# zkp-gravity/0g-halo2

Measured on AMD Instinct MI355X. Metric: create_proof proofs/hour, model_28input_256entry_1hash_1bpi, higher is better.
Workload: dtype u32x8 (254-bit Montgomery integers)

## Files before the change

### 0g-halo2_amd/csrc/field9.h

```cpp
#pragma once

#include "curve.h"
#include "field.h"

namespace zg {

struct F9 {
    int32_t l[9];
};

constexpr int32_t MASK29 = (1 << 29) - 1;

struct Fq9Params {
    static __device__ __forceinline__ int32_t p(int i) {
        constexpr int32_t P[9] = {0x187cfd47, 0x010460b6, 0x1c72a34f, 0x02d522d0, 0x1585d978,
                                  0x02db40c0, 0x00a6e141, 0x0e5c2634, 0x0030644e};
        return P[i];
    }
    static constexpr uint32_t INV29 = 0x04866389u;
    static __device__ __forceinline__ F9 one() {
        return F9{{0x157ccc21, 0x141c2758, 0x185230d3, 0x014c0419, 0x0aa36fb9, 0x1d4240ce, 0x11d54c07, 0x052ac7a8, 0x000dc836}};
    }
    static __device__ __forceinline__ F9 k256() {
        return F9{{0x058f0d9d, 0x1aea1c6e, 0x11c2cf74, 0x11d651eb, 0x1462c0a7, 0x11b7bc3c, 0x1cbd99ba, 0x183340fb, 0x000e0a77}};
// ... 284 lines not shown
        c = w >> 29;
    }
    a.l[8] = (int32_t)((int64_t)v.l[8] - (int64_t)q * (int64_t)P::p(8) + c);
    int32_t b = 0;
#pragma unroll
    for (int i = 0; i < 8; i++) {
        const int32_t w = a.l[i] - P::p(i) + b;
        t.l[i] = w & MASK29;
        b = w >> 29;
    }
    t.l[8] = a.l[8] - P::p(8) + b;
    const bool ge = t.l[8] >= 0;
#pragma unroll
    for (int i = 0; i < 9; i++) a.l[i] = ge ? t.l[i] : a.l[i];
    return f9_pack(a);
}

struct alignas(16) XYZZ9 {
    F9 x, y, zz, zzz;
};
static_assert(sizeof(XYZZ9) == 144, "XYZZ9 layout");

__device__ __forceinline__ XYZZ9 xyzz9_identity() {
    XYZZ9 r;
#pragma unroll
    for (int i = 0; i < 9; i++) r.x.l[i] = r.y.l[i] = r.zz.l[i] = r.zzz.l[i] = 0;
    return r;
}
__device__ __forceinline__ bool xyzz9_is_identity(const XYZZ9& a) { return f9_limbs_zero(a.zz); }

// ... 332 lines not shown
```

### 0g-halo2_amd/csrc/poly.h

```cpp
#pragma once

#include "common.h"
#include "msm.h"

namespace zg {

struct alignas(16) DMono {
    Fe coeff;
    uint32_t n_factors;
    uint32_t coeff_is_one;
    uint32_t factors[ZG_MAX_FACTORS];
    uint32_t pad[2];
};
static_assert(sizeof(DMono) == 80, "DMono layout");

struct DLookup {
    uint32_t width;
    zg_poly inputs[ZG_MAX_LOOKUP_WIDTH];
    zg_poly tables[ZG_MAX_LOOKUP_WIDTH];
};

struct DevCircuit {
    const zg_query* queries;
    const DMono* monos;
    const zg_poly* gates;
    const DLookup* lookups;
    const zg_query* perm_cols;
    uint32_t n_gates, n_lookups, n_perm, chunk, n_sets;
};

struct Cols {
    const Fe* fixed;
    const Fe* advice;
    const Fe* instance;
    uint32_t log_size;
    int32_t rot_scale;
    size_t adv_bs, inst_bs;
};

constexpr uint32_t PC_MAX_POINTS = 16;
constexpr uint32_t EH_MAX_YPOW = 48;
struct alignas(16) ProofConst {
    uint32_t key[8];
    Fe theta, beta, gamma;
    Fe eh_y, eh_beta, eh_gamma, eh_theta;
    Fe eh_delta_start[2];
    Fe eh_ypow[EH_MAX_YPOW];
    Fe xn;
    Fe v;
    Fe points[PC_MAX_POINTS];
    Fe subs[PC_MAX_POINTS];
};

struct EvalHArgs {
    DevCircuit c;
    Cols cols;
    const Fe* sigma_cos;
    const Fe* pz_cos;
    const Fe* lz_cos;
    const Fe* pin_cos;
    const Fe* ptab_cos;
    size_t perm_stride;
    const Fe* l0;
    const Fe* llast;
    const Fe* lactive;
    const Fe* ext_tw;
    const Fe* t_eval;
    uint32_t t_mask;
    int32_t last_rot;
    const ProofConst* pc;
    uint32_t zpow;
    size_t cos_bs, h_bs;
// ... 110 lines not shown
```

### 0g-halo2_amd/csrc/poly.hip

```cpp
#include "poly.h"
#include "poly_eval.h"
#include "field9.h"

namespace zg {

__host__ __device__ __forceinline__ uint32_t rotl32(uint32_t x, int sft) { return (x << sft) | (x >> (32 - sft)); }
#define ZG_QR(a, b, c, d)                       \
    do {                                        \
        a += b; d ^= a; d = rotl32(d, 16);      \
        c += d; b ^= c; b = rotl32(b, 12);      \
        a += b; d ^= a; d = rotl32(d, 8);       \
        c += d; b ^= c; b = rotl32(b, 7);       \
    } while (0)

__host__ __device__ inline Fe rand_fr(const uint32_t* key, uint32_t tag, uint64_t index) {
    Fe v;
    for (uint32_t attempt = 0;; attempt++) {
        uint32_t x0 = 0x61707865u, x1 = 0x3320646eu, x2 = 0x79622d32u, x3 = 0x6b206574u;
        uint32_t x4 = key[0], x5 = key[1], x6 = key[2], x7 = key[3], x8 = key[4], x9 = key[5], x10 = key[6], x11 = key[7];
        uint32_t x12 = attempt, x13 = tag, x14 = (uint32_t)index, x15 = (uint32_t)(index >> 32);
        for (int r = 0; r < 10; r++) {
            ZG_QR(x0, x4, x8, x12);
            ZG_QR(x1, x5, x9, x13);
            ZG_QR(x2, x6, x10, x14);
// ... 668 lines not shown
#pragma unroll
    for (int i = 0; i < 9; i++) acc.l[i] = 0;
    uint32_t pending = 0;
    auto add = [&](const F9& t, bool neg) {
        acc = neg ? f9_sub(acc, t) : f9_add(acc, t);
        if (++pending == 2) {
            acc = f9_norm(acc);
            pending = 0;
        }
    };
    F9 hl, hr;
    bool held = false, hneg = false;
    for (uint32_t m = p.first; m < p.first + p.count; m++) {
        const DMono* mo = monos + m;
        const uint32_t nf = mo->n_factors;
        const bool unit = mo->coeff_is_one != 0 && nf > 0;
        const bool neg = unit && mo->coeff_is_one == 2;
        const uint32_t terms = nf + (unit ? 0u : 1u);
        if (terms == 1) {
            add(unit ? cell(mo->factors[0]) : f9_unpack(mo->coeff), neg);
            continue;
        }
        uint32_t f = 0;
        F9 l = unit ? cell(mo->factors[f++]) : f9_unpack(mo->coeff);
        for (; f + 1 < nf; f++) l = Fr9::mul(l, cell(mo->factors[f]));
        const F9 r = cell(mo->factors[nf - 1]);
        if (held) {
            if (hneg == neg) add(Fr9::mul2<false>(hl, hr, l, r), neg);
            else add(Fr9::mul2<true>(hl, hr, l, r), hneg);
            held = false;
        } else {
            hl = l;
            hr = r;
            hneg = neg;
            held = true;
        }
    }
    if (held) add(Fr9::mul(hl, hr), hneg);
    return f9_norm(acc);
// ... 9 lines not shown
                                                           const Fe* __restrict__ coef, uint32_t count, Fe* __restrict__ out) {
    const uint32_t idx = blockIdx.x * blockDim.x + threadIdx.x;
    if (idx >= en) return;
    stg(out + idx, f9_reduce_pack<Fr9Params>(horner9(ld9(col + ((idx + rot_off) & (en - 1))), coef, count)));
}

int poly_gate_factor(zg_ctx* ctx, const Fe* col, uint32_t rot_off, uint32_t en, const Fe* coef, uint32_t count, Fe* out) {
    ZG_REQUIRE(count >= 1 && (en & (en - 1)) == 0, ZG_ERR_INVALID_ARG, "poly_gate_factor: %u coefficients, %u points", count, en);
    ZG_LAUNCH(ctx, "gate_factor", 2.0 * en * 32.0, gate_factor9_kernel, dim3((en + 255) / 256), dim3(256), 0, col, rot_off, en, coef,
              count, out);
    ZG_HIP(hipGetLastError());
    return ZG_OK;
}

template <bool GROUPED>
__global__ __launch_bounds__(256) void evaluate_h9_kernel(EvalHArgs a, uint32_t en) {
    const uint32_t idx = blockIdx.x * blockDim.x + threadIdx.x;
    if (idx >= en) return;
    const EvalHProof pr = evalh_proof(a, blockIdx.y);
    const ProofConst* pc = pr.pc;
    const DevCircuit& c = a.c;
    const uint32_t mask = en - 1;
    const uint32_t rs = (uint32_t)a.cols.rot_scale;
    const uint32_t r_next = (idx + rs) & mask;
    const uint32_t r_prev = (idx - rs) & mask;
    const uint32_t r_last = (idx + (uint32_t)(a.last_rot * (int32_t)rs)) & mask;
    auto fold = [&](const F9& value, const F9& term) { return f9_add(Fr9::mul(value, f9_unpack(pc->eh_y)), term); };
    auto fold2 = [&](const F9& value, const F9& u, const F9& v) { return Fr9::mul2<false>(value, f9_unpack(pc->eh_y), u, v); };
    F9 value;
#pragma unroll
    for (int i = 0; i < 9; i++) value.l[i] = 0;
    auto cell = [&](uint32_t qi) {
        const zg_query q = c.queries[qi];
        const Fe* base = q.kind == ZG_FIXED ? pr.cols.fixed : q.kind == ZG_ADVICE ? pr.cols.advice : pr.cols.instance;
// ... 40 lines not shown
        for (int i = 0; i < 9; i++) s0.l[i] = sl.l[i] = sa.l[i] = 0;
        auto acc1 = [&](F9& s, uint32_t e, const F9& t) { s = f9_norm(f9_add(s, Fr9::mul(yw(e), t))); };
        auto acc2 = [&](F9& s, uint32_t e, const F9& t, uint32_t e2, const F9& t2) {
            s = f9_norm(f9_add(s, Fr9::mul2<false>(yw(e), t, yw(e2), t2)));
        };
        if (c.n_sets > 0) {
            const F9 zf = ld9(pr.pz_cos + idx);
            const F9 zl = ld9(pr.pz_cos + (size_t)(c.n_sets - 1) * en + idx);
            acc1(s0, w - 1, f9_sub(one(), zf));
            acc1(sl, w - 2, f9_sub(Fr9::sqr(zl), zl));
            w -= 2;
            for (uint32_t s = 1; s < c.n_sets; s++) {
                const F9 t = f9_sub(ld9(pr.pz_cos + (size_t)s * en + idx), ld9(pr.pz_cos + (size_t)(s - 1) * en + r_last));
                acc1(s0, --w, t);
            }
            F9 current_delta = Fr9::mul(f9_unpack(pc->eh_delta_start[a.zpow - 1]), ld9(a.ext_tw + idx));
            const F9 delta = f9_unpack(a.delta);
            for (uint32_t s = 0; s < c.n_sets; s++) {
                uint32_t c0 = s * c.chunk, c1 = c0 + c.chunk;
                if (c1 > c.n_perm) c1 = c.n_perm;
                F9 left = ld9(pr.pz_cos + (size_t)s * en + r_next);
                F9 right = ld9(pr.pz_cos + (size_t)s * en + idx);
                for (uint32_t col = c0; col < c1; col++) {
                    const zg_query q = c.perm_cols[col];
                    const Fe* base = q.kind == ZG_FIXED ? pr.cols.fixed : q.kind == ZG_ADVICE ? pr.cols.advice : pr.cols.instance;
                    const F9 v = ld9(base + ((size_t)q.column << a.cols.log_size) + idx);
                    const F9 sg = ld9(a.sigma_cos + (size_t)col * en + idx);
                    const F9 fl = f9_norm(f9_add(f9_add(Fr9::mul(f9_unpack(pc->eh_beta), sg), v), f9_unpack(pc->eh_gamma)));
                    const F9 fr = f9_norm(f9_add(f9_add(v, current_delta), f9_unpack(pc->eh_gamma)));
                    current_delta = Fr9::mul(current_delta, delta);
                    if (col + 1 < c1) {
                        left = Fr9::mul(left, fl);
                        right = Fr9::mul(right, fr);
                    } else {
                        left = Fr9::mul2<true>(left, fl, right, fr);
                    }
                }
                acc1(sa, --w, left);
            }
        }
        for (uint32_t l = 0; l < c.n_lookups; l++) {
            const DLookup* lk = c.lookups + l;
            F9 ai, ti;
            compress(lk, ai, ti);
            const Fe* zc = pr.lz_cos + (size_t)l * en;
            const Fe* ap = pr.pin_cos + (size_t)l * a.perm_stride;
            const Fe* sp = pr.ptab_cos + (size_t)l * a.perm_stride;
            const F9 z = ld9(zc + idx), apv = ld9(ap + idx), spv = ld9(sp + idx);
            const F9 lft = Fr9::mul(f9_add(apv, f9_unpack(pc->eh_beta)), f9_norm(f9_add(spv, f9_unpack(pc->eh_gamma))));
            const F9 rgt = Fr9::mul(f9_norm(f9_add(ai, f9_unpack(pc->eh_beta))), f9_norm(f9_add(ti, f9_unpack(pc->eh_gamma))));
            const F9 ams = f9_sub(apv, spv);
            acc2(s0, w - 1, f9_sub(one(), z), w - 4, ams);
            acc1(sl, w - 2, f9_sub(Fr9::sqr(z), z));
// ... 57 lines not shown
    value = Fr9::mul(value, ld9(a.t_eval + (idx & a.t_mask)));
    stg(pr.h + idx, f9_reduce_pack<Fr9Params>(value));
}

int poly_evaluate_h(zg_ctx* ctx, const EvalHArgs& a, uint32_t en, uint32_t nb, uint32_t n_columns, double unit_share) {
    if (!nb) return ZG_OK;
    ZG_REQUIRE(a.pc != nullptr && (a.zpow == 1 || a.zpow == 2), ZG_ERR_INVALID_ARG, "evaluate_h: per-proof scalars missing");
    const DevCircuit& c = a.c;
    const double arrays = (double)n_columns + 3.0 + c.n_perm + c.n_sets + 3.0 * c.n_lookups + 1.0;
    const double unit = nb * arrays * unit_share * 32.0;
    ZG_REQUIRE(!a.hat || a.monos_hat != nullptr || (c.n_gates == 0 && c.n_lookups == 0), ZG_ERR_INVALID_ARG,
               "evaluate_h: the 2^261-form monomial table is missing");
    ZG_REQUIRE(!a.hat || c.n_gates == 0 || (a.gates_hat != nullptr && a.gate_common != nullptr && a.gate_uni != nullptr && a.uni_coef != nullptr && a.gate_slab != nullptr && a.gate_slabs != nullptr), ZG_ERR_INVALID_ARG,
               "evaluate_h: the factored gate table is missing");
    if (a.hat && a.n_terms)
        ZG_LAUNCH_U(ctx, "evaluate_h", nb * arrays * en * 32.0, unit, evaluate_h9_kernel<true>, dim3((en + 255) / 256, nb), dim3(256), 0, a, en);
    else if (a.hat)
        ZG_LAUNCH_U(ctx, "evaluate_h", nb * arrays * en * 32.0, unit, evaluate_h9_kernel<false>, dim3((en + 255) / 256, nb), dim3(256), 0, a, en);
    else
        ZG_LAUNCH_U(ctx, "evaluate_h", nb * arrays * en * 32.0, unit, evaluate_h_kernel, dim3((en + 255) / 256, nb), dim3(256), 0, a, en);
    ZG_HIP(hipGetLastError());
    return ZG_OK;
}

__device__ __forceinline__ const Fe* poly_of(const PolySet& ps, uint32_t ix, uint32_t b) {
    return ix < ps.nsh ? ps.sh + (size_t)ix * ps.n : ps.pp + (size_t)b * ps.pp_bs + (size_t)(ix - ps.nsh) * ps.n;
}

template <uint32_t CH>
__global__ __launch_bounds__(256) void powers_kernel(const ProofConst* __restrict__ pc, uint32_t n, Fe* __restrict__ pw,
                                                     size_t pw_bs) {
    uint32_t i0 = (blockIdx.x * blockDim.x + threadIdx.x) * CH;
    if (i0 >= n) return;
// ... 524 lines not shown
```

### 0g-halo2_amd/csrc/prove_batch.hip

```cpp
#include <algorithm>
#include <chrono>

#include "prover.h"
#include "field9.h"
#include "transcript.h"

using namespace zg;

namespace {

Fe rotate_omega(const PkDev& k, const Fe& x, int32_t rot) {
    Fe w = rot >= 0 ? Fr::pow_u64(k.omega, (uint64_t)rot) : Fr::pow_u64(k.omega_inv, (uint64_t)(-(int64_t)rot));
    return Fr::mul(x, w);
}

constexpr int LAT_GATE_DEFAULT = 0;
constexpr int LAT_PULL_DEFAULT = 1;
void* stage(zg_prover* p, const void* src, size_t bytes) {
    void* dst = p->pin.stage_take(bytes);
    if (dst) memcpy(dst, src, bytes);
    return dst;
}
int h2d_list(zg_prover* p, uint32_t* d_dst, const std::vector<uint32_t>& list) {
    std::vector<uint32_t>& held = p->uploaded_lists[d_dst];
// ... 509 lines not shown
        const uint32_t mb = S + NL;
        if (mb) {
            ZG_TRY(wait_points(p, (size_t)nb * prod_per, pts, W_PRODUCTS));
            ZG_TICK("products: points on the host");
            for (uint32_t b = 0; b < nb; b++) {
                const Jac* q = &pts[(size_t)b * prod_per];
                for (uint32_t i = 0; i < mb; i++) tr[b].write_point(q[i]);
                if (!have_random) random_commit[b] = q[mb];
            }
        } else if (!have_random) {
            ZG_TRY(wait_points(p, nb, pts, W_PRODUCTS));
            for (uint32_t b = 0; b < nb; b++) random_commit[b] = pts[b];
        }
        have_random = true;
        for (uint32_t b = 0; b < nb; b++) tr[b].write_point(random_commit[b]);
        for (uint32_t b = 0; b < nb; b++) evalh_consts(p->hpc[b], tr[b].squeeze(), hat, evalh_terms(pk));
        ZG_TICK("y");
        ZG_TRY(publish());
        ZG_TICK("y uploaded");
        lap(2);
        return ZG_OK;
    }

    int quotient_queue() {
        ZG_TRY(join());
        if (!phase_cosets) ZG_TRY(to_cosets(ctx, p->ix_adv, p->ncos));
        for (uint32_t di = dlo; di < dhi; di++) {
            const EvalHArgs a = evalh_args(p, di);
            ZG_TRY(poly_evaluate_h(ctx, a, pk.dom[di].en, nb, A + I + pk.F, (double)((size_t)1 << ek) * ((double)pk.dom[di].en / parts_en)));
        }
        p->have_last = true;
// ... 306 lines not shown
```

### 0g-halo2_amd/csrc/prover.h

```cpp
#pragma once

#include <memory>

#include "poly.h"
#include "check.h"

namespace zg {

struct PkDev {
    int device = 0;
    uint32_t k = 0, ext_k = 0, cs_degree = 0, bf = 0, qpd = 0;
    uint32_t n = 0, en = 0, usable = 0;
    uint32_t F = 0, A = 0, I = 0, P = 0, NL = 0, sets = 0, chunk = 0;
    std::vector<zg_query> advice_queries, fixed_queries;
    DevCircuit dc{};
    std::vector<void*> owned;
    bool hat = true;
    bool grouped = true;
    DMono* monos_hat = nullptr;
    zg_poly* gates_hat = nullptr;
    uint32_t* gate_common = nullptr;
    zg_poly* gate_uni = nullptr;
    Fe* uni_coef = nullptr;
    uint32_t* gate_slab = nullptr;
    struct SlabJob { uint32_t gate, query, first, count; };
    std::vector<SlabJob> slab_jobs;
    Fe vk_repr{};
    Fe omega{}, omega_inv{}, ifft_div{};
    Fe *fixed_val = nullptr, *sigma_val = nullptr, *omega_tw = nullptr;
    Fe* sh_polys = nullptr;
    struct Dom {
        uint32_t ek = 0, en = 0;
        int zpow = 1;
        Fe *fixed_cos = nullptr, *sigma_cos = nullptr, *l0 = nullptr, *llast = nullptr, *lactive = nullptr,
           *gate_slabs = nullptr, *t_eval = nullptr, *ext_tw = nullptr;
    };
    Dom dom[3];
    uint32_t nparts = 1;
    uint32_t NG = 0;
    CheckInfo ck;
    ~PkDev() {
        (void)hipSetDevice(device);
        for (void* q : owned) (void)hipFree(q);
    }
};

struct PinnedArena {
    static constexpr size_t MARGIN = 4096;
    char* host = nullptr;
// ... 75 lines not shown
    zg::PinnedArena pin;
    bool have_last = false;
    bool in_flight = false;
    bool last_split = false;
    uint32_t last_nb = 0;
    double phase_ms[8] = {0, 0, 0, 0, 0, 0, 0, 0};
};

namespace zg {

int prover_drain(zg_prover* p);
int batch_args_ok(const char* who, const char* what, const zg_prover* p, size_t count, const zg_fr* const* instance, size_t instance_len);
int advice_into_slots(zg_prover* p, uint32_t nb, const zg_fr* const* advice_host, void* const* advice_dev);
int upload_consts(zg_prover* p, uint32_t nb);
uint32_t evalh_terms(const PkDev& pk);
void evalh_consts(ProofConst& c, const Fe& y, bool hat, uint32_t n_terms);
EvalHArgs evalh_args(const zg_prover* p, uint32_t di);
int shard_gather_sum(zg_prover* p, size_t count, XYZZ* out);

}
```

### 0g-halo2_amd/csrc/prover.hip

```cpp
#include <algorithm>
#include <cstdlib>
#include <memory>

#include "prover.h"
#include "field9.h"

using namespace zg;

namespace {

constexpr int LAT_SPLIT_K_DEFAULT = 15;

template <class T>
int dalloc_into(std::vector<void*>& owned, T** out, size_t count) {
    void* q = nullptr;
    size_t bytes = (count ? count : 1) * sizeof(T);
    hipError_t e = hipMalloc(&q, bytes);
    if (e != hipSuccess) {
        set_error("zg_prover: hipMalloc(%zu) failed: %s", bytes, hipGetErrorString(e));
        return ZG_ERR_OOM;
    }
    owned.push_back(q);
    *out = reinterpret_cast<T*>(q);
    return ZG_OK;
// ... 9 lines not shown
static bool lone_split(const zg_prover* p, bool latency_form) {
    const int sk = knob(K_LAT_SPLIT_K);
    return latency_form && p->pk->k >= (uint32_t)(sk >= 0 ? sk : LAT_SPLIT_K_DEFAULT);
}

}

namespace zg {

uint32_t evalh_terms(const PkDev& pk) {
    const bool grouped = pk.grouped;
    const uint32_t t = (pk.sets ? 2 + (pk.sets - 1) + pk.sets : 0) + 5 * pk.NL;
    return grouped && pk.hat && t >= 1 && t <= 40 && t + 1 <= EH_MAX_YPOW ? t : 0;
}

void evalh_consts(ProofConst& c, const Fe& y, bool hat, uint32_t n_terms) {
    const Fe zeta = fr_zeta(), zeta2 = Fr::sqr(zeta);
    c.eh_y = y; c.eh_beta = c.beta; c.eh_gamma = c.gamma; c.eh_theta = c.theta;
    c.eh_delta_start[0] = Fr::mul(c.beta, zeta);
    c.eh_delta_start[1] = Fr::mul(c.beta, zeta2);
    if (hat) {
        const Fe c261 = Fr9Params::c261_fe();
        for (Fe* cst : {&c.eh_y, &c.eh_beta, &c.eh_gamma, &c.eh_theta, &c.eh_delta_start[0], &c.eh_delta_start[1]})
            *cst = Fr::mul(*cst, c261);
        Fe pw = Fr::one();
        for (uint32_t j = 0; j <= n_terms && j < EH_MAX_YPOW; j++) {
            c.eh_ypow[j] = Fr::mul(pw, c261);
            pw = Fr::mul(pw, y);
        }
    }
}

EvalHArgs evalh_args(const zg_prover* p, uint32_t di) {
    const PkDev& pk = *p->pk;
    const uint32_t n = pk.n, k = pk.k, bf = pk.bf, A = pk.A, I = pk.I, NL = pk.NL, S = pk.sets;
    const bool hat = pk.hat;
    const PkDev::Dom& d = pk.dom[di];
    const Fe* cos = p->dbuf[di].cos;
    EvalHArgs a;
    memset(&a, 0, sizeof(a));
    a.c = pk.dc;
    a.cols.fixed = d.fixed_cos; a.cols.advice = cos; a.cols.instance = cos + (size_t)A * d.en;
    a.cols.log_size = d.ek; a.cols.rot_scale = (int32_t)(d.en / n);
    a.cols.adv_bs = a.cols.inst_bs = (size_t)p->ncos * d.en;
    a.sigma_cos = d.sigma_cos;
    a.pz_cos = cos + (size_t)(A + I) * d.en;
    a.lz_cos = a.pz_cos + (size_t)S * d.en;
    a.pin_cos = a.lz_cos + (size_t)NL * d.en; a.ptab_cos = a.pin_cos + d.en; a.perm_stride = (size_t)2 * d.en;
    a.l0 = d.l0; a.llast = d.llast; a.lactive = d.lactive;
    a.ext_tw = hat ? d.ext_tw + d.en : d.ext_tw;
    a.t_eval = d.t_eval; a.t_mask = (1u << (d.ek - k)) - 1;
    a.last_rot = -(int32_t)(bf + 1);
    a.pc = p->d_pc; a.zpow = (uint32_t)d.zpow;
    a.cos_bs = (size_t)p->ncos * d.en; a.h_bs = d.en;
    a.delta = hat ? Fr::mul(fr_delta(), Fr9Params::c261_fe()) : fr_delta();
    a.hat = hat;
    a.monos_hat = pk.monos_hat;
    a.n_terms = evalh_terms(pk);
    a.gates_hat = pk.gates_hat;
    a.gate_common = pk.gate_common;
// ... 72 lines not shown
    ZG_TRY(dalloc_into(own, &p->d_idx, (size_t)4 * p->max_evals + 64 + (size_t)p->max_points * 512));
    ZG_TRY(dalloc_into(own, &p->ktmp, poly_kate_tmp_elems(n, cap * p->max_points)));
    ZG_TRY(dalloc_into(own, &p->d_pc, c));
    p->hpc.assign(cap, ProofConst{});
    PinnedArena& pin = p->pin;
    pin.evals_at = (c * p->maxv * sizeof(XYZZ) + 4095) & ~size_t(4095);
    pin.errors_at = pin.evals_at + c * p->max_evals * sizeof(Fe);
    pin.stage_begin = pin.evals_at + ((c * p->max_evals * sizeof(Fe) + c * NL * 4 + 4095) & ~size_t(4095));
    pin.cap = pin.stage_begin + (1u << 20) + c * 16 * sizeof(ProofConst) + c * (size_t)k.I * 4096;
    ZG_HIP(hipHostMalloc((void**)&pin.host, pin.cap, hipHostMallocMapped | hipHostMallocCoherent));
    ZG_HIP(hipHostGetDevicePointer((void**)&pin.dev, pin.host, 0));
    memset(pin.host + pin.stage_end(), 0, PinnedArena::MARGIN);
    return ZG_OK;
}

struct GateFactor {
    std::vector<DMono> inner;
    std::vector<Fe> uc;
    uint32_t cost = 0;
};

GateFactor factor_gate(const std::vector<DMono>& monos, zg_poly g, uint32_t f, const Fe& c261, bool tabulated) {
    auto strip = [&](const DMono& src, bool all) {
        DMono d = src;
        uint32_t w = 0;
        bool dropped = false;
        for (uint32_t b = 0; b < src.n_factors; b++) {
            if (src.factors[b] == f && (all || !dropped)) { dropped = true; continue; }
            d.factors[w++] = src.factors[b];
        }
// ... 29 lines not shown
            univariate = grp.size() == base.size();
            for (size_t i = 0; i < grp.size() && univariate; i++)
                univariate = same_cells(grp[i], base[i]) &&
                             fe_eq(Fr::mul(grp[i].coeff, base[0].coeff), Fr::mul(grp[0].coeff, base[i].coeff));
            if (univariate) out.uc[k - 1] = Fr::mul(Fr::mul(grp[0].coeff, b0_inv), c261);
        }
        if (univariate) {
            size_t best = 0, best_n = 0;
            for (size_t i = 0; i < base.size(); i++) {
                size_t cnt = 0;
                const Fe neg_i = Fr::neg(base[i].coeff);
                for (const DMono& o : base) cnt += fe_eq(o.coeff, base[i].coeff) || fe_eq(o.coeff, neg_i);
                if (cnt > best_n) best = i, best_n = cnt;
            }
            const Fe d = base[best].coeff, d_inv = Fr::inv(d);
            const Fe one_hat = Fr::mul(Fr::one(), c261);
            for (DMono& o : base) {
                o.coeff = Fr::mul(Fr::mul(o.coeff, d_inv), c261);
                o.coeff_is_one = fe_eq(o.coeff, one_hat) ? 1 : fe_eq(o.coeff, Fr::neg(one_hat)) ? 2 : 0;
            }
            for (Fe& u : out.uc) u = Fr::mul(u, Fr::mul(d, Fr::inv(c261)));
            out.inner = std::move(base);
        }
    }
    if (!univariate) {
        out.uc.clear();
        for (uint32_t m = g.first; m < g.first + g.count; m++) out.inner.push_back(strip(monos[m], false));
    }
    for (const DMono& d : out.inner) {
        const uint32_t operands = d.n_factors + (d.coeff_is_one && d.n_factors ? 0u : 1u);
        out.cost += operands ? operands - 1 : 0;
    }
    if (!out.uc.empty() && !tabulated) out.cost += (uint32_t)out.uc.size();
    return out;
// ... 22 lines not shown
    ZG_REQUIRE(pk->ext_k <= 22, ZG_ERR_UNSUPPORTED, "zg_prover_create: extended domain 2^%u not built", pk->ext_k);
    pk->en = 1u << pk->ext_k;
    ZG_REQUIRE(pk->n > pk->bf + 2, ZG_ERR_INVALID_ARG, "zg_prover_create: too few rows");
    pk->usable = pk->n - (pk->bf + 1);
    pk->F = cs->n_fixed; pk->A = cs->n_advice; pk->I = cs->n_instance; pk->P = cs->n_perm_columns; pk->NL = cs->n_lookups;
    pk->chunk = cs->cs_degree - 2;
    pk->sets = pk->P ? (pk->P + pk->chunk - 1) / pk->chunk : 0;
    pk->advice_queries.assign(cs->advice_queries, cs->advice_queries + cs->n_advice_queries);
    pk->fixed_queries.assign(cs->fixed_queries, cs->fixed_queries + cs->n_fixed_queries);
    pk->vk_repr = to_fe(vk_repr);
    pk->omega = host_domain_omega(pk->k);
    pk->omega_inv = Fr::inv(pk->omega);
    pk->ifft_div = Fr::inv(Fr::from_u64(pk->n));
    pk->hat = knob(K_EVALH9) != 0;
    pk->grouped = knob(K_EVALH_GROUPED) != 0;
    return ZG_OK;
}

int validate_circuit(const PkDev* pk, const zg_circuit* cs, std::vector<DMono>& monos, std::vector<DLookup>& lks) {
    for (uint32_t q = 0; q < cs->n_queries; q++) {
        const zg_query& qq = cs->queries[q];
        uint32_t lim = qq.kind == ZG_FIXED ? pk->F : qq.kind == ZG_ADVICE ? pk->A : qq.kind == ZG_INSTANCE ? pk->I : 0;
        ZG_REQUIRE(qq.column < lim, ZG_ERR_INVALID_ARG, "zg_prover_create: query %u names column %u of kind %u", q,
                   qq.column, qq.kind);
    }
    monos.assign(cs->n_monomials, DMono{});
    Fe one = Fr::one();
    for (uint32_t m = 0; m < cs->n_monomials; m++) {
        const zg_monomial& s = cs->monomials[m];
        ZG_REQUIRE(s.n_factors <= ZG_MAX_FACTORS, ZG_ERR_INVALID_ARG, "zg_prover_create: monomial %u has %u factors", m, s.n_factors);
// ... 70 lines not shown
    for (uint32_t a = 0; a < first.n_factors; a++) {
        const uint32_t cand = first.factors[a];
        if (a && cand == first.factors[a - 1]) continue;
        bool all = true;
        for (uint32_t m = g.first; m < g.first + g.count && all; m++)
            all = std::find(monos[m].factors, monos[m].factors + monos[m].n_factors, cand) != monos[m].factors + monos[m].n_factors;
        if (!all) continue;
        GateFactor opt = factor_gate(monos, g, cand, c261, cs->queries[cand].kind == ZG_FIXED);
        if (*f == 0xffffffffu || opt.cost < best.cost) best = std::move(opt), *f = cand;
    }
    return best;
}

int factored_view(PkDev* pk, const zg_circuit* cs, std::vector<DMono>& monos) {
    const Fe c261 = Fr9Params::c261_fe();
    for (auto& d : monos) d.coeff = Fr::mul(d.coeff, c261);
    std::vector<zg_poly> gates_hat(cs->n_gates);
    std::vector<uint32_t> common(cs->n_gates, 0xffffffffu);
    std::vector<zg_poly> gate_uni(cs->n_gates, zg_poly{0, 0});
    std::vector<Fe> uni_coef;
    for (uint32_t gi = 0; gi < cs->n_gates; gi++) {
        const zg_poly g = cs->gates[gi];
        gates_hat[gi] = g;
        if (g.count < 2) continue;
        uint32_t f;
        const GateFactor best = cheapest_factor(monos, cs, g, c261, &f);
        if (f == 0xffffffffu) continue;
        gates_hat[gi].first = (uint32_t)monos.size();
        gates_hat[gi].count = (uint32_t)best.inner.size();
        monos.insert(monos.end(), best.inner.begin(), best.inner.end());
        if (!best.uc.empty()) {
            gate_uni[gi].first = (uint32_t)uni_coef.size();
            gate_uni[gi].count = (uint32_t)best.uc.size();
            if (cs->queries[f].kind == ZG_FIXED) pk->slab_jobs.push_back({gi, f, gate_uni[gi].first, gate_uni[gi].count});
            uni_coef.insert(uni_coef.end(), best.uc.begin(), best.uc.end());
        }
        common[gi] = f;
    }
    ZG_TRY(key_alloc(pk, &pk->gate_uni, cs->n_gates ? cs->n_gates : 1));
    ZG_TRY(key_alloc(pk, &pk->uni_coef, uni_coef.size() ? uni_coef.size() : 1));
    if (cs->n_gates) ZG_HIP(hipMemcpy(pk->gate_uni, gate_uni.data(), cs->n_gates * sizeof(zg_poly), hipMemcpyHostToDevice));
    if (!uni_coef.empty()) ZG_HIP(hipMemcpy(pk->uni_coef, uni_coef.data(), uni_coef.size() * sizeof(Fe), hipMemcpyHostToDevice));
    ZG_TRY(key_alloc(pk, &pk->monos_hat, monos.size() ? monos.size() : 1));
    ZG_TRY(key_alloc(pk, &pk->gates_hat, cs->n_gates ? cs->n_gates : 1));
    ZG_TRY(key_alloc(pk, &pk->gate_common, cs->n_gates ? cs->n_gates : 1));
    if (!monos.empty()) ZG_HIP(hipMemcpy(pk->monos_hat, monos.data(), monos.size() * sizeof(DMono), hipMemcpyHostToDevice));
    if (cs->n_gates) {
        ZG_HIP(hipMemcpy(pk->gates_hat, gates_hat.data(), cs->n_gates * sizeof(zg_poly), hipMemcpyHostToDevice));
        ZG_HIP(hipMemcpy(pk->gate_common, common.data(), cs->n_gates * sizeof(uint32_t), hipMemcpyHostToDevice));
    }
    return ZG_OK;
}

// ... 61 lines not shown
        pk->nparts = 3;
        pk->dom[1].ek = pk->k + log2u(m1); pk->dom[1].en = n * m1; pk->dom[1].zpow = 1;
        pk->dom[2].ek = pk->k + log2u(m2); pk->dom[2].en = n * m2; pk->dom[2].zpow = 2;
    }
}

int alloc_key_slabs(PkDev* pk) {
    const uint32_t n = pk->n, F = pk->F, P = pk->P;
    ZG_TRY(key_alloc(pk, &pk->sh_polys, (size_t)(F + P) * n));
    ZG_TRY(key_alloc(pk, &pk->fixed_val, (size_t)F * n));
    ZG_TRY(key_alloc(pk, &pk->sigma_val, (size_t)P * n));
    for (uint32_t di = 0; di < pk->nparts; di++) {
        PkDev::Dom& d = pk->dom[di];
        ZG_TRY(key_alloc(pk, &d.fixed_cos, (size_t)F * d.en));
        ZG_TRY(key_alloc(pk, &d.sigma_cos, (size_t)P * d.en));
        ZG_TRY(key_alloc(pk, &d.l0, (size_t)d.en));
        ZG_TRY(key_alloc(pk, &d.llast, (size_t)d.en));
        ZG_TRY(key_alloc(pk, &d.lactive, (size_t)d.en));
    }
    return ZG_OK;
}

int key_columns(zg_ctx* ctx, PkDev* pk, const zg_fr* values, uint32_t count, Fe* val, Fe* polys, Fe* PkDev::Dom::*cos) {
    const uint32_t n = pk->n;
    if (!count) return ZG_OK;
    ZG_HIP(hipMemcpyAsync(val, values, (size_t)count * n * 32, hipMemcpyHostToDevice, ctx->stream));
    ZG_TRY(ntt_batch_to_dev(ctx, val, polys, n, count, pk->k, pk->omega_inv, &pk->ifft_div));
    for (uint32_t di = 0; di < pk->nparts; di++) {
        PkDev::Dom& d = pk->dom[di];
        ZG_TRY(coeff_to_coset_dev(ctx, polys, n, n, d.*cos, d.en, count, d.ek, pk->hat, d.zpow));
    }
    return ZG_OK;
}

int key_gate_slabs(zg_ctx* ctx, PkDev* pk, const zg_circuit* cs) {
    const uint32_t n = pk->n;
    hipStream_t st = ctx->stream;
    std::vector<uint32_t> slab_of(cs->n_gates ? cs->n_gates : 1, 0xffffffffu);
    ZG_TRY(key_alloc(pk, &pk->gate_slab, slab_of.size()));
    for (uint32_t di = 0; di < pk->nparts; di++) {
        PkDev::Dom& d = pk->dom[di];
        ZG_TRY(key_alloc(pk, &d.gate_slabs, std::max<size_t>(1, pk->slab_jobs.size() * (size_t)d.en)));
        for (size_t j = 0; j < pk->slab_jobs.size(); j++) {
            const auto& job = pk->slab_jobs[j];
            const zg_query q = cs->queries[job.query];
// ... 131 lines not shown
    ZG_TRY(prover_events(p));
    if (p->use_side && !ctx->side) ZG_TRY(zg_ctx_create(ctx->device, &ctx->side));
    std::vector<DMono> monos;
    std::vector<DLookup> lks;
    ZG_TRY(validate_circuit(pk, cs, monos, lks));
    check_info(pk, cs, monos, lks);
    ZG_TRY(upload_circuit(pk, cs, monos, lks, ctx->stream));
    if (pk->hat) ZG_TRY(factored_view(pk, cs, monos));
    ZG_TRY(attach_bases(p, g, g_lagrange, shared_g, shared_gl));
    ZG_TRY(enable_tables(p));
    choose_domain_parts(pk);
    ZG_TRY(alloc_key_slabs(pk));
    ZG_TRY(key_columns(ctx, pk, fixed_values, pk->F, pk->fixed_val, pk->sh_polys, &PkDev::Dom::fixed_cos));
    if (pk->hat) ZG_TRY(key_gate_slabs(ctx, pk, cs));
    ZG_TRY(key_columns(ctx, pk, sigma_values, pk->P, pk->sigma_val, pk->sh_polys + (size_t)pk->F * pk->n, &PkDev::Dom::sigma_cos));
    ZG_TRY(key_l_polynomials(ctx, pk));
    ZG_TRY(key_t_evals(ctx, pk));
    ZG_HIP(hipStreamSynchronize(ctx->stream));
    p->lat_split = lone_split(p, p->use_side);
    ZG_TRY(alloc_slots(p, 1));
    *out = guard.release();
    return ZG_OK;
}

int zg_prover_create(zg_ctx* ctx, const zg_circuit* cs, const zg_fr* fixed_values, const zg_fr* sigma_values,
                     const zg_g1_affine* g, const zg_g1_affine* g_lagrange, const zg_fr* vk_repr, zg_prover** out) {
    ZG_REQUIRE(g && g_lagrange, ZG_ERR_INVALID_ARG, "zg_prover_create: null SRS");
    return prover_create_impl(ctx, cs, fixed_values, sigma_values, g, g_lagrange, nullptr, nullptr, vk_repr, out);
}

// ... 165 lines not shown
    ZG_REQUIRE(p->cap >= 1, ZG_ERR_INVALID_ARG, "zg_prover_evaluate_h: the prover has no slot");
    zg_ctx* ctx = p->ctx;
    ZG_ENTER(ctx);
    hipStream_t st = ctx->stream;
    const uint32_t n = pk.n;
    p->have_last = false;
    struct Fam { const zg_fr* src; uint32_t ix, count; };
    const Fam fams[] = {{advice_polys, p->ix_adv, pk.A}, {instance_polys, p->ix_inst, pk.I}, {perm_z_polys, p->ix_pz, pk.sets},
                        {lookup_z_polys, p->ix_lz, pk.NL}, {permuted_polys, p->ix_perm, 2 * pk.NL}};
    for (const Fam& f : fams)
        if (f.count)
            ZG_HIP(hipMemcpyAsync(p->pp + (size_t)(f.ix - p->nsh) * n, f.src, (size_t)f.count * n * 32, hipMemcpyHostToDevice, st));
    ProofConst& c = p->hpc[0];
    memset(&c, 0, sizeof(c));
    c.theta = to_fe(theta); c.beta = to_fe(beta); c.gamma = to_fe(gamma);
    evalh_consts(c, to_fe(y), pk.hat, evalh_terms(pk));
    p->pin.stage_reset();
    ZG_TRY(upload_consts(p, 1));
    const PkDev::Dom& d = pk.dom[0];
    ZG_TRY(coeff_to_coset_dev(ctx, p->pp + (size_t)(p->ix_adv - p->nsh) * n, n, n, p->dbuf[0].cos, d.en, p->ncos, d.ek, pk.hat, d.zpow));
    const EvalHArgs a = evalh_args(p, 0);
    ZG_TRY(poly_evaluate_h(ctx, a, d.en, 1, pk.A + pk.I + pk.F, (double)d.en));
    WsScope ws(ctx);
    Fe* tmp = ws.get<Fe>(d.en);
    if (!tmp) return ZG_ERR_OOM;
    ZG_TRY(poly_scale(ctx, p->dbuf[0].h, tmp, d.en, pk.hat ? Fr::inv(Fr::from_u64(32)) : Fr::one()));
    ZG_HIP(hipMemcpyAsync(h_out, tmp, (size_t)d.en * 32, hipMemcpyDeviceToHost, st));
    ZG_HIP(hipStreamSynchronize(st));
    return ZG_OK;
}

// ... 33 lines not shown
```

Baseline: 5.183 million.

## Prescale permutation sigma columns, use small-integer coefficient multiplies, remap evaluate_h grid

Precomputes sigma columns scaled by shift and delta inverses at key time. The permutation argument in evaluate_h then needs one multiply per column instead of a beta multiply plus a running delta multiply, and per-set products are folded into precomputed y-power constants. Gate monomials whose coefficients are small integers use a cheap float-estimated small-multiply reduction instead of a full Montgomery multiply. The evaluate_h grid is flattened with proofs interleaved and block indices swizzled across 8 groups. The cost is extra device memory for the scaled sigma columns, more per-proof host constant work, and correctness that depends on the float quotient estimate.

```diff
diff --git a/0g-halo2_amd/csrc/field9.h b/0g-halo2_amd/csrc/field9.h
--- a/0g-halo2_amd/csrc/field9.h
+++ b/0g-halo2_amd/csrc/field9.h
@@ -322,6 +322,23 @@
 #pragma unroll
     for (int i = 0; i < 9; i++) a.l[i] = ge ? t.l[i] : a.l[i];
     return f9_pack(a);
+}
+
+constexpr int32_t F9_SMALL_MAX = 1 << 12;
+template <class P>
+__device__ __forceinline__ F9 f9_mul_small(const F9& x, int32_t c) {
+    const float top = (float)x.l[8] + (float)x.l[7] * 1.862645149230957e-09f;
+    const int32_t q = (int32_t)floorf(top * (float)c * 3.153175148504101e-07f - 0.05f);
+    F9 a;
+    int64_t cy = 0;
+#pragma unroll
+    for (int i = 0; i < 8; i++) {
+        const int64_t w = (int64_t)x.l[i] * (int64_t)c - (int64_t)q * (int64_t)P::p(i) + cy;
+        a.l[i] = (int32_t)((uint32_t)w & (uint32_t)MASK29);
+        cy = w >> 29;
+    }
+    a.l[8] = (int32_t)((int64_t)x.l[8] * (int64_t)c - (int64_t)q * (int64_t)P::p(8) + cy);
+    return a;
 }
 
 struct alignas(16) XYZZ9 {
diff --git a/0g-halo2_amd/csrc/poly.h b/0g-halo2_amd/csrc/poly.h
--- a/0g-halo2_amd/csrc/poly.h
+++ b/0g-halo2_amd/csrc/poly.h
@@ -10,7 +10,8 @@
     uint32_t n_factors;
     uint32_t coeff_is_one;
     uint32_t factors[ZG_MAX_FACTORS];
-    uint32_t pad[2];
+    int32_t small;
+    uint32_t pad;
 };
 static_assert(sizeof(DMono) == 80, "DMono layout");
 
@@ -40,12 +41,16 @@
 
 constexpr uint32_t PC_MAX_POINTS = 16;
 constexpr uint32_t EH_MAX_YPOW = 48;
+constexpr uint32_t EH_MAX_PCOLS = 16, EH_MAX_PSETS = 8;
 struct alignas(16) ProofConst {
     uint32_t key[8];
     Fe theta, beta, gamma;
     Fe eh_y, eh_beta, eh_gamma, eh_theta;
     Fe eh_delta_start[2];
     Fe eh_ypow[EH_MAX_YPOW];
+    Fe eh_pcol[2][EH_MAX_PCOLS];
+    Fe eh_pw[2][EH_MAX_PSETS];
+    uint32_t eh_scaled, eh_pad[7];
     Fe xn;
     Fe v;
     Fe points[PC_MAX_POINTS];
@@ -56,6 +61,7 @@
     DevCircuit c;
     Cols cols;
     const Fe* sigma_cos;
+    const Fe* sigma_sc;
     const Fe* pz_cos;
     const Fe* lz_cos;
     const Fe* pin_cos;
diff --git a/0g-halo2_amd/csrc/poly.hip b/0g-halo2_amd/csrc/poly.hip
--- a/0g-halo2_amd/csrc/poly.hip
+++ b/0g-halo2_amd/csrc/poly.hip
@@ -706,15 +706,20 @@
     for (uint32_t m = p.first; m < p.first + p.count; m++) {
         const DMono* mo = monos + m;
         const uint32_t nf = mo->n_factors;
-        const bool unit = mo->coeff_is_one != 0 && nf > 0;
-        const bool neg = unit && mo->coeff_is_one == 2;
+        const uint32_t kind = mo->coeff_is_one;
+        const bool small = kind == 3 && nf > 0;
+        const bool unit = (kind == 1 || kind == 2 || small) && nf > 0;
+        const bool neg = kind == 2 && nf > 0;
         const uint32_t terms = nf + (unit ? 0u : 1u);
         if (terms == 1) {
-            add(unit ? cell(mo->factors[0]) : f9_unpack(mo->coeff), neg);
+            F9 t = unit ? cell(mo->factors[0]) : f9_unpack(mo->coeff);
+            if (small) t = f9_mul_small<Fr9Params>(t, mo->small);
+            add(t, neg);
             continue;
         }
         uint32_t f = 0;
         F9 l = unit ? cell(mo->factors[f++]) : f9_unpack(mo->coeff);
+        if (small) l = f9_mul_small<Fr9Params>(l, mo->small);
         for (; f + 1 < nf; f++) l = Fr9::mul(l, cell(mo->factors[f]));
         const F9 r = cell(mo->factors[nf - 1]);
         if (held) {
@@ -754,10 +759,13 @@
 }
 
 template <bool GROUPED>
-__global__ __launch_bounds__(256) void evaluate_h9_kernel(EvalHArgs a, uint32_t en) {
-    const uint32_t idx = blockIdx.x * blockDim.x + threadIdx.x;
+__global__ __launch_bounds__(256) void evaluate_h9_kernel(EvalHArgs a, uint32_t en, uint32_t nb) {
+    uint32_t bid = blockIdx.x;
+    if ((gridDim.x & 7u) == 0) bid = (bid & 7u) * (gridDim.x >> 3) + (bid >> 3);
+    const uint32_t tile = bid / nb;
+    const uint32_t idx = tile * blockDim.x + threadIdx.x;
     if (idx >= en) return;
-    const EvalHProof pr = evalh_proof(a, blockIdx.y);
+    const EvalHProof pr = evalh_proof(a, bid - tile * nb);
     const ProofConst* pc = pr.pc;
     const DevCircuit& c = a.c;
     const uint32_t mask = en - 1;
@@ -828,8 +836,9 @@
                 const F9 t = f9_sub(ld9(pr.pz_cos + (size_t)s * en + idx), ld9(pr.pz_cos + (size_t)(s - 1) * en + r_last));
                 acc1(s0, --w, t);
             }
-            F9 current_delta = Fr9::mul(f9_unpack(pc->eh_delta_start[a.zpow - 1]), ld9(a.ext_tw + idx));
-            const F9 delta = f9_unpack(a.delta);
+            const bool scaled = a.sigma_sc != nullptr && pc->eh_scaled != 0;
+            F9 current_delta = ld9(a.ext_tw + idx);
+            if (!scaled) current_delta = Fr9::mul(f9_unpack(pc->eh_delta_start[a.zpow - 1]), current_delta);
             for (uint32_t s = 0; s < c.n_sets; s++) {
                 uint32_t c0 = s * c.chunk, c1 = c0 + c.chunk;
                 if (c1 > c.n_perm) c1 = c.n_perm;
@@ -839,18 +848,26 @@
                     const zg_query q = c.perm_cols[col];
                     const Fe* base = q.kind == ZG_FIXED ? pr.cols.fixed : q.kind == ZG_ADVICE ? pr.cols.advice : pr.cols.instance;
                     const F9 v = ld9(base + ((size_t)q.column << a.cols.log_size) + idx);
-                    const F9 sg = ld9(a.sigma_cos + (size_t)col * en + idx);
-                    const F9 fl = f9_norm(f9_add(f9_add(Fr9::mul(f9_unpack(pc->eh_beta), sg), v), f9_unpack(pc->eh_gamma)));
-                    const F9 fr = f9_norm(f9_add(f9_add(v, current_delta), f9_unpack(pc->eh_gamma)));
-                    current_delta = Fr9::mul(current_delta, delta);
+                    F9 fl, fr;
+                    if (scaled) {
+                        const F9 t = Fr9::mul(f9_add(v, f9_unpack(pc->eh_gamma)), f9_unpack(pc->eh_pcol[a.zpow - 1][col]));
+                        fl = f9_add(ld9(a.sigma_sc + (size_t)col * en + idx), t);
+                        fr = f9_add(current_delta, t);
+                    } else {
+                        const F9 sg = ld9(a.sigma_cos + (size_t)col * en + idx);
+                        fl = f9_norm(f9_add(f9_add(Fr9::mul(f9_unpack(pc->eh_beta), sg), v), f9_unpack(pc->eh_gamma)));
+                        fr = f9_norm(f9_add(f9_add(v, current_delta), f9_unpack(pc->eh_gamma)));
+                        current_delta = Fr9::mul(current_delta, f9_unpack(a.delta));
+                    }
                     if (col + 1 < c1) {
                         left = Fr9::mul(left, fl);
                         right = Fr9::mul(right, fr);
                     } else {
-                        left = Fr9::mul2<true>(left, fl, right, fr);
+                        left = Fr9::mul2<true>(left, f9_norm(fl), right, f9_norm(fr));
                     }
                 }
-                acc1(sa, --w, left);
+                --w;
+                sa = f9_norm(f9_add(sa, Fr9::mul(scaled ? f9_unpack(pc->eh_pw[a.zpow - 1][s]) : yw(w), left)));
             }
         }
         for (uint32_t l = 0; l < c.n_lookups; l++) {
@@ -938,9 +955,9 @@
     ZG_REQUIRE(!a.hat || c.n_gates == 0 || (a.gates_hat != nullptr && a.gate_common != nullptr && a.gate_uni != nullptr && a.uni_coef != nullptr && a.gate_slab != nullptr && a.gate_slabs != nullptr), ZG_ERR_INVALID_ARG,
                "evaluate_h: the factored gate table is missing");
     if (a.hat && a.n_terms)
-        ZG_LAUNCH_U(ctx, "evaluate_h", nb * arrays * en * 32.0, unit, evaluate_h9_kernel<true>, dim3((en + 255) / 256, nb), dim3(256), 0, a, en);
+        ZG_LAUNCH_U(ctx, "evaluate_h", nb * arrays * en * 32.0, unit, evaluate_h9_kernel<true>, dim3((en + 255) / 256 * nb), dim3(256), 0, a, en, nb);
     else if (a.hat)
-        ZG_LAUNCH_U(ctx, "evaluate_h", nb * arrays * en * 32.0, unit, evaluate_h9_kernel<false>, dim3((en + 255) / 256, nb), dim3(256), 0, a, en);
+        ZG_LAUNCH_U(ctx, "evaluate_h", nb * arrays * en * 32.0, unit, evaluate_h9_kernel<false>, dim3((en + 255) / 256 * nb), dim3(256), 0, a, en, nb);
     else
         ZG_LAUNCH_U(ctx, "evaluate_h", nb * arrays * en * 32.0, unit, evaluate_h_kernel, dim3((en + 255) / 256, nb), dim3(256), 0, a, en);
     ZG_HIP(hipGetLastError());
diff --git a/0g-halo2_amd/csrc/prove_batch.hip b/0g-halo2_amd/csrc/prove_batch.hip
--- a/0g-halo2_amd/csrc/prove_batch.hip
+++ b/0g-halo2_amd/csrc/prove_batch.hip
@@ -547,7 +547,7 @@
         }
         have_random = true;
         for (uint32_t b = 0; b < nb; b++) tr[b].write_point(random_commit[b]);
-        for (uint32_t b = 0; b < nb; b++) evalh_consts(p->hpc[b], tr[b].squeeze(), hat, evalh_terms(pk));
+        for (uint32_t b = 0; b < nb; b++) evalh_consts(p->hpc[b], tr[b].squeeze(), pk);
         ZG_TICK("y");
         ZG_TRY(publish());
         ZG_TICK("y uploaded");
diff --git a/0g-halo2_amd/csrc/prover.h b/0g-halo2_amd/csrc/prover.h
--- a/0g-halo2_amd/csrc/prover.h
+++ b/0g-halo2_amd/csrc/prover.h
@@ -26,13 +26,13 @@
     struct SlabJob { uint32_t gate, query, first, count; };
     std::vector<SlabJob> slab_jobs;
     Fe vk_repr{};
-    Fe omega{}, omega_inv{}, ifft_div{};
+    Fe omega{}, omega_inv{}, ifft_div{}, delta_inv{};
     Fe *fixed_val = nullptr, *sigma_val = nullptr, *omega_tw = nullptr;
     Fe* sh_polys = nullptr;
     struct Dom {
         uint32_t ek = 0, en = 0;
         int zpow = 1;
-        Fe *fixed_cos = nullptr, *sigma_cos = nullptr, *l0 = nullptr, *llast = nullptr, *lactive = nullptr,
+        Fe *fixed_cos = nullptr, *sigma_cos = nullptr, *sigma_sc = nullptr, *l0 = nullptr, *llast = nullptr, *lactive = nullptr,
            *gate_slabs = nullptr, *t_eval = nullptr, *ext_tw = nullptr;
     };
     Dom dom[3];
@@ -138,7 +138,8 @@
 int advice_into_slots(zg_prover* p, uint32_t nb, const zg_fr* const* advice_host, void* const* advice_dev);
 int upload_consts(zg_prover* p, uint32_t nb);
 uint32_t evalh_terms(const PkDev& pk);
-void evalh_consts(ProofConst& c, const Fe& y, bool hat, uint32_t n_terms);
+bool evalh_perm_scaled(const PkDev& pk);
+void evalh_consts(ProofConst& c, const Fe& y, const PkDev& pk);
 EvalHArgs evalh_args(const zg_prover* p, uint32_t di);
 int shard_gather_sum(zg_prover* p, size_t count, XYZZ* out);
 
diff --git a/0g-halo2_amd/csrc/prover.hip b/0g-halo2_amd/csrc/prover.hip
--- a/0g-halo2_amd/csrc/prover.hip
+++ b/0g-halo2_amd/csrc/prover.hip
@@ -47,19 +47,47 @@
     return grouped && pk.hat && t >= 1 && t <= 40 && t + 1 <= EH_MAX_YPOW ? t : 0;
 }
 
-void evalh_consts(ProofConst& c, const Fe& y, bool hat, uint32_t n_terms) {
+bool evalh_perm_scaled(const PkDev& pk) {
+    return evalh_terms(pk) != 0 && pk.P >= 1 && pk.P <= EH_MAX_PCOLS && pk.sets <= EH_MAX_PSETS;
+}
+
+void evalh_consts(ProofConst& c, const Fe& y, const PkDev& pk) {
+    const bool hat = pk.hat;
+    const uint32_t n_terms = evalh_terms(pk);
     const Fe zeta = fr_zeta(), zeta2 = Fr::sqr(zeta);
     c.eh_y = y; c.eh_beta = c.beta; c.eh_gamma = c.gamma; c.eh_theta = c.theta;
     c.eh_delta_start[0] = Fr::mul(c.beta, zeta);
     c.eh_delta_start[1] = Fr::mul(c.beta, zeta2);
+    c.eh_scaled = 0;
     if (hat) {
         const Fe c261 = Fr9Params::c261_fe();
         for (Fe* cst : {&c.eh_y, &c.eh_beta, &c.eh_gamma, &c.eh_theta, &c.eh_delta_start[0], &c.eh_delta_start[1]})
             *cst = Fr::mul(*cst, c261);
+        Fe ypw[EH_MAX_YPOW];
         Fe pw = Fr::one();
         for (uint32_t j = 0; j <= n_terms && j < EH_MAX_YPOW; j++) {
+            ypw[j] = pw;
             c.eh_ypow[j] = Fr::mul(pw, c261);
             pw = Fr::mul(pw, y);
+        }
+        if (evalh_perm_scaled(pk) && !fe_is_zero(c.beta)) {
+            const Fe shift[2] = {zeta, zeta2}, shift_inv[2] = {zeta2, zeta};
+            const Fe beta_inv = Fr::inv(c.beta), delta = fr_delta();
+            Fe dpow = Fr::one(), dipow = Fr::one();
+            for (uint32_t s = 0; s < pk.sets; s++) {
+                Fe prod[2] = {Fr::one(), Fr::one()};
+                for (uint32_t col = s * pk.chunk; col < std::min(pk.P, (s + 1) * pk.chunk); col++) {
+                    for (int a = 0; a < 2; a++) {
+                        c.eh_pcol[a][col] = Fr::mul(Fr::mul(Fr::mul(beta_inv, dipow), shift_inv[a]), c261);
+                        prod[a] = Fr::mul(prod[a], Fr::mul(Fr::mul(c.beta, dpow), shift[a]));
+                    }
+                    dpow = Fr::mul(dpow, delta);
+                    dipow = Fr::mul(dipow, pk.delta_inv);
+                }
+                const uint32_t e = n_terms - pk.sets - 2 - s;
+                for (int a = 0; a < 2; a++) c.eh_pw[a][s] = Fr::mul(Fr::mul(ypw[e], prod[a]), c261);
+            }
+            c.eh_scaled = 1;
         }
     }
 }
@@ -77,6 +105,7 @@
     a.cols.log_size = d.ek; a.cols.rot_scale = (int32_t)(d.en / n);
     a.cols.adv_bs = a.cols.inst_bs = (size_t)p->ncos * d.en;
     a.sigma_cos = d.sigma_cos;
+    a.sigma_sc = d.sigma_sc;
     a.pz_cos = cos + (size_t)(A + I) * d.en;
     a.lz_cos = a.pz_cos + (size_t)S * d.en;
     a.pin_cos = a.lz_cos + (size_t)NL * d.en; a.ptab_cos = a.pin_cos + d.en; a.perm_stride = (size_t)2 * d.en;
@@ -179,6 +208,29 @@
     return ZG_OK;
 }
 
+void classify_coeff9(DMono& d) {
+    const Fe raw_one{{1, 0, 0, 0, 0, 0, 0, 0}};
+    const Fe unhat = Fr::inv(Fr::from_u64(32));
+    auto small_int = [&](const Fe& hat, int32_t* out) {
+        const Fe v = Fr::mul(Fr::mul(hat, unhat), raw_one);
+        for (int i = 1; i < 8; i++)
+            if (v.l[i]) return false;
+        *out = (int32_t)v.l[0];
+        return v.l[0] <= (uint32_t)F9_SMALL_MAX;
+    };
+    int32_t c = 0;
+    d.small = 0;
+    if (small_int(d.coeff, &c)) {
+        d.coeff_is_one = c == 1 ? 1 : 3;
+        d.small = c;
+    } else if (small_int(Fr::neg(d.coeff), &c)) {
+        d.coeff_is_one = c == 1 ? 2 : 3;
+        d.small = -c;
+    } else {
+        d.coeff_is_one = 0;
+    }
+}
+
 struct GateFactor {
     std::vector<DMono> inner;
     std::vector<Fe> uc;
@@ -238,10 +290,9 @@
                 if (cnt > best_n) best = i, best_n = cnt;
             }
             const Fe d = base[best].coeff, d_inv = Fr::inv(d);
-            const Fe one_hat = Fr::mul(Fr::one(), c261);
             for (DMono& o : base) {
                 o.coeff = Fr::mul(Fr::mul(o.coeff, d_inv), c261);
-                o.coeff_is_one = fe_eq(o.coeff, one_hat) ? 1 : fe_eq(o.coeff, Fr::neg(one_hat)) ? 2 : 0;
+                classify_coeff9(o);
             }
             for (Fe& u : out.uc) u = Fr::mul(u, Fr::mul(d, Fr::inv(c261)));
             out.inner = std::move(base);
@@ -294,6 +345,7 @@
     pk->ifft_div = Fr::inv(Fr::from_u64(pk->n));
     pk->hat = knob(K_EVALH9) != 0;
     pk->grouped = knob(K_EVALH_GROUPED) != 0;
+    pk->delta_inv = Fr::inv(fr_delta());
     return ZG_OK;
 }
 
@@ -394,7 +446,10 @@
 
 int factored_view(PkDev* pk, const zg_circuit* cs, std::vector<DMono>& monos) {
     const Fe c261 = Fr9Params::c261_fe();
-    for (auto& d : monos) d.coeff = Fr::mul(d.coeff, c261);
+    for (auto& d : monos) {
+        d.coeff = Fr::mul(d.coeff, c261);
+        classify_coeff9(d);
+    }
     std::vector<zg_poly> gates_hat(cs->n_gates);
     std::vector<uint32_t> common(cs->n_gates, 0xffffffffu);
     std::vector<zg_poly> gate_uni(cs->n_gates, zg_poly{0, 0});
@@ -417,6 +472,25 @@
         }
         common[gi] = f;
     }
+#ifdef ZG_TICKS
+    {
+        uint32_t full = 0, small = 0, cells = 0;
+        auto tally = [&](zg_poly q) {
+            for (uint32_t m = q.first; m < q.first + q.count; m++) {
+                const DMono& d = monos[m];
+                if (!d.n_factors) continue;
+                full += d.coeff_is_one == 0;
+                small += d.coeff_is_one == 3;
+                cells += d.n_factors - 1;
+            }
+        };
+        for (uint32_t gi = 0; gi < cs->n_gates; gi++) tally(gates_hat[gi]);
+        for (uint32_t l = 0; l < cs->n_lookups; l++)
+            for (uint32_t e = 0; e < cs->lookups[l].width; e++) tally(cs->lookups[l].inputs[e]), tally(cs->lookups[l].tables[e]);
+        fprintf(stderr, "evaluate_h tables: per row %u products by a full coefficient, %u by a small integer, %u between cells\n",
+                full, small, cells);
+    }
+#endif
     ZG_TRY(key_alloc(pk, &pk->gate_uni, cs->n_gates ? cs->n_gates : 1));
     ZG_TRY(key_alloc(pk, &pk->uni_coef, uni_coef.size() ? uni_coef.size() : 1));
     if (cs->n_gates) ZG_HIP(hipMemcpy(pk->gate_uni, gate_uni.data(), cs->n_gates * sizeof(zg_poly), hipMemcpyHostToDevice));
@@ -508,6 +582,7 @@
         PkDev::Dom& d = pk->dom[di];
         ZG_TRY(key_alloc(pk, &d.fixed_cos, (size_t)F * d.en));
         ZG_TRY(key_alloc(pk, &d.sigma_cos, (size_t)P * d.en));
+        if (evalh_perm_scaled(*pk)) ZG_TRY(key_alloc(pk, &d.sigma_sc, (size_t)P * d.en));
         ZG_TRY(key_alloc(pk, &d.l0, (size_t)d.en));
         ZG_TRY(key_alloc(pk, &d.llast, (size_t)d.en));
         ZG_TRY(key_alloc(pk, &d.lactive, (size_t)d.en));
@@ -523,6 +598,20 @@
     for (uint32_t di = 0; di < pk->nparts; di++) {
         PkDev::Dom& d = pk->dom[di];
         ZG_TRY(coeff_to_coset_dev(ctx, polys, n, n, d.*cos, d.en, count, d.ek, pk->hat, d.zpow));
+    }
+    return ZG_OK;
+}
+
+int key_sigma_scaled(zg_ctx* ctx, PkDev* pk) {
+    if (!evalh_perm_scaled(*pk)) return ZG_OK;
+    const Fe zeta = fr_zeta(), zeta2 = Fr::sqr(zeta);
+    for (uint32_t di = 0; di < pk->nparts; di++) {
+        PkDev::Dom& d = pk->dom[di];
+        Fe f = d.zpow == 1 ? zeta2 : zeta;
+        for (uint32_t col = 0; col < pk->P; col++) {
+            ZG_TRY(poly_scale(ctx, d.sigma_cos + (size_t)col * d.en, d.sigma_sc + (size_t)col * d.en, d.en, f));
+            f = Fr::mul(f, pk->delta_inv);
+        }
     }
     return ZG_OK;
 }
@@ -684,6 +773,7 @@
     ZG_TRY(key_columns(ctx, pk, fixed_values, pk->F, pk->fixed_val, pk->sh_polys, &PkDev::Dom::fixed_cos));
     if (pk->hat) ZG_TRY(key_gate_slabs(ctx, pk, cs));
     ZG_TRY(key_columns(ctx, pk, sigma_values, pk->P, pk->sigma_val, pk->sh_polys + (size_t)pk->F * pk->n, &PkDev::Dom::sigma_cos));
+    ZG_TRY(key_sigma_scaled(ctx, pk));
     ZG_TRY(key_l_polynomials(ctx, pk));
     ZG_TRY(key_t_evals(ctx, pk));
     ZG_HIP(hipStreamSynchronize(ctx->stream));
@@ -879,7 +969,7 @@
     ProofConst& c = p->hpc[0];
     memset(&c, 0, sizeof(c));
     c.theta = to_fe(theta); c.beta = to_fe(beta); c.gamma = to_fe(gamma);
-    evalh_consts(c, to_fe(y), pk.hat, evalh_terms(pk));
+    evalh_consts(c, to_fe(y), pk);
     p->pin.stage_reset();
     ZG_TRY(upload_consts(p, 1));
     const PkDev::Dom& d = pk.dom[0];
```

New measurement: 5.278 million, median of 6. 1.8% higher.
